# yavuzmurattas/Infrared-Colorization-with-ResNet-Generator-and-PatchGAN

Measured on AMD Instinct MI355X. Metric: GAN train-step img/s (G+D fwd/bwd) at 256×256, 1/2/4/8 MI355X, higher is better.
Workload: dtype bf16; 1 GPU; GAN train step 256x256, batch 16/GPU, bf16 (BASELINE configs[1]); global_batch=16, img_size=256, height=256, width=256, parallelism=dp1

## Files before the change

### include/irgan.h

```cpp
#ifndef IRGAN_H
#define IRGAN_H
#include <stdint.h>
#include <stddef.h>

#if defined(__GNUC__) || defined(__clang__)
#define IRGAN_API __attribute__((visibility("default")))
#else
#define IRGAN_API
#endif

#ifdef __cplusplus
extern "C" {
#endif

typedef void* irgan_stream_t;

IRGAN_API int irgan_build_id(char* buf, int32_t len);

enum { IRGAN_F32 = 0, IRGAN_BF16 = 1, IRGAN_FP8 = 2 };
enum { IRGAN_PAD_ZERO = 0, IRGAN_PAD_REFLECT = 1 };
enum { IRGAN_ACT_NONE = 0, IRGAN_ACT_RELU = 1, IRGAN_ACT_LRELU = 2, IRGAN_ACT_TANH = 3 };
enum { IRGAN_OK = 0, IRGAN_EINVAL = 1001, IRGAN_EUNSUPPORTED = 1002 };

typedef struct irgan_conv_desc {
// ... 31 lines not shown
IRGAN_API int irgan_fp8_quant(const void* x, int32_t dt, int64_t P, int32_t C, int32_t ldx, int32_t xoff,
                    void* y, int32_t ldy, int32_t yoff, const float* q, uint32_t* amax,
                    irgan_stream_t s);
IRGAN_API int irgan_fp8_scale(uint32_t* amax, int32_t n, float* q, float* dq, int32_t reset, irgan_stream_t s);
typedef struct irgan_fp8_job {
    const void* src;
    void* dst;
    int64_t n;
    int32_t slot, reserved;
} irgan_fp8_job;
IRGAN_API int irgan_fp8_quant_batch(const void* jobs, int32_t njobs, int64_t max_n, const float* q,
                          uint32_t* amax, irgan_stream_t s);

IRGAN_API int irgan_conv_fwd_splitk(const irgan_conv_desc* d, const void* x, const void* w, float* y,
                          int32_t ksplit, int64_t split_stride, irgan_stream_t s);

IRGAN_API int irgan_conv_wgrad(const irgan_conv_desc* d, const void* x, const void* dy,
                     float* dw, int32_t splitk, irgan_stream_t s);

IRGAN_API int irgan_conv_wgrad_ws(const irgan_conv_desc* d, const void* x, const void* dy, float* dw,
                        int32_t splitk, float* ws, int64_t ws_floats, irgan_stream_t s);

IRGAN_API int irgan_weight_pack(const float* src, void* dst, int32_t dtype, int32_t Cout, int32_t KH,
                      int32_t KW, int32_t Cin, int32_t transpose, int32_t s, int32_t tyr,
                      int32_t Ay, int32_t txr, int32_t Ax, int32_t cpad, int32_t kalign,
                      irgan_stream_t st);

typedef struct irgan_pack_desc {
    const float* src;
    void* dst;
    int32_t dtype, Cout, KH, KW, Cin, transpose, s, tyr, Ay, txr, Ax, cpad, kalign, reserved;
} irgan_pack_desc;
IRGAN_API int irgan_weight_pack_batch(const irgan_pack_desc* descs, int32_t n, irgan_stream_t st);

enum { IRGAN_IN_PARTS = 256 };
IRGAN_API int irgan_in_finalize(const void* part, int32_t N, int32_t HW, int32_t C, int32_t nb, float* mr,
                      irgan_stream_t s);
IRGAN_API int irgan_in_stats(const void* x, int32_t dtype, int32_t N, int32_t HW, int32_t C,
                   int32_t ld, int32_t off, double* work, float* mr, irgan_stream_t s);
IRGAN_API int irgan_in_apply(const void* x, int32_t dtype, int32_t N, int32_t HW, int32_t C, int32_t ldx,
                   int32_t xoff, const float* mr, int32_t act, const void* res, int32_t ldr,
                   int32_t roff, void* y, int32_t ldy, int32_t yoff, void* xhat, irgan_stream_t s);
IRGAN_API int irgan_in_bwd_reduce(const void* dy, int32_t dy_dtype, int32_t lddy, int32_t dyoff,
                        const void* dy2, int32_t dy2_dtype, int32_t lddy2, int32_t dy2off,
                        const void* x, int32_t x_dtype, int32_t ldx, int32_t xoff, int32_t act,
                        int32_t N, int32_t HW, int32_t C, const float* mr, double* work,
                        float* red, irgan_stream_t s);
IRGAN_API int irgan_in_bwd_apply(const void* dy, int32_t dy_dtype, int32_t lddy, int32_t dyoff,
                       const void* dy2, int32_t dy2_dtype, int32_t lddy2, int32_t dy2off,
                       const void* x, int32_t x_dtype, int32_t ldx, int32_t xoff, int32_t act,
                       int32_t N, int32_t HW, int32_t C, const float* mr, const float* red,
                       void* dx, int32_t dx_dtype, int32_t lddx, int32_t dxoff, float* db,
                       irgan_stream_t s);

IRGAN_API int irgan_in_apply_fp8(const void* x, int32_t N, int32_t HW, int32_t C, int32_t ldx, int32_t xoff,
                       const float* mr, int32_t act, const void* res, int32_t ldr, int32_t roff, void* y,
                       int32_t ldy, int32_t yoff, void* y8, int32_t ld8, int32_t off8, const float* q,
                       uint32_t* amax, irgan_stream_t s);
IRGAN_API int irgan_in_bwd_apply_fp8(const void* dy, int32_t lddy, int32_t dyoff, const void* dy2, int32_t lddy2,
                           int32_t dy2off, const void* x, int32_t ldx, int32_t xoff, int32_t act, int32_t N,
                           int32_t HW, int32_t C, const float* mr, const float* red, void* dx, int32_t lddx,
                           int32_t dxoff, void* y8, int32_t ld8, int32_t off8, const float* q,
                           uint32_t* amax, irgan_stream_t s);
IRGAN_API int irgan_channel_sum(const void* g, int32_t dtype, int32_t P, int32_t C, int32_t ld,
                      int32_t off, float* db, double* work, irgan_stream_t s);

enum { IRGAN_BN_TABLE = 4 };
enum { IRGAN_NORM_AFFINE = 256 };
IRGAN_API int irgan_bn_finalize(const void* part, int32_t N, int32_t HW, int32_t C, int32_t nb, int32_t G,
                      const float* gamma, const float* beta, float* running_mean, float* running_var,
                      float momentum, float eps, int32_t repeat, float* mr, float* ab, irgan_stream_t s);
IRGAN_API int irgan_bn_stats(const void* x, int32_t dtype, int32_t N, int32_t HW, int32_t C, int32_t ld,
                   int32_t off, int32_t G, const float* gamma, const float* beta, float* running_mean,
                   float* running_var, float momentum, float eps, int32_t repeat, double* work, float* mr,
                   float* ab, irgan_stream_t s);
IRGAN_API int irgan_bn_eval_table(const float* running_mean, const float* running_var, const float* gamma,
                        const float* beta, int32_t N, int32_t C, float eps, float* mr, float* ab,
                        irgan_stream_t s);
IRGAN_API int irgan_bn_apply(const void* x, int32_t dtype, int32_t N, int32_t HW, int32_t C, int32_t ldx,
                   int32_t xoff, const float* mr, const float* gamma, const float* beta, int32_t act,
                   const void* res, int32_t ldr, int32_t roff, void* y, int32_t ldy, int32_t yoff,
                   irgan_stream_t s);
IRGAN_API int irgan_bn_backward(const void* dy, int32_t dy_dtype, int32_t lddy, int32_t dyoff, const void* dy2,
                      int32_t dy2_dtype, int32_t lddy2, int32_t dy2off, const void* x, int32_t x_dtype,
                      int32_t ldx, int32_t xoff, int32_t act, int32_t N, int32_t HW, int32_t C, int32_t G,
                      int32_t eval, const float* mr, const float* gamma, const float* beta, double* work,
                      float* red, void* dx, int32_t dx_dtype, int32_t lddx, int32_t dxoff, float* dgamma,
                      float* dbeta, irgan_stream_t s);

IRGAN_API int irgan_resample_table(int32_t kind, int32_t n_in, int32_t p, int32_t transpose, int32_t* idx,
                         float* w, int32_t tmax, int32_t rows_cap);
IRGAN_API int irgan_reflect_ring_fold(const float* rows, const float* cols, int32_t nsplit, int32_t N, int32_t H,
                            int32_t W, int32_t C, int32_t p, void* dx, int32_t dx_dtype, int32_t lddx,
                            int32_t dxoff, irgan_stream_t s);
IRGAN_API int irgan_reflect_dgrad_ring(const irgan_conv_desc* d, const void* dy, const void* w, int32_t p, void* dx,
                             irgan_stream_t s);
IRGAN_API int irgan_reflect_dgrad_ring_ws(const irgan_conv_desc* d, const void* dy, const void* w, int32_t p, void* dx,
                                float* ws, int64_t ws_floats, int32_t max_blocks, irgan_stream_t s);
IRGAN_API int irgan_conv_dgrad_reflect_line(const irgan_conv_desc* d, const void* dy, const void* w, int32_t p, void* dx,
                                  float* ws, int64_t ws_floats, irgan_stream_t s);
IRGAN_API int irgan_conv_dgrad_reflect_line_fp8(const irgan_conv_desc* d, const void* dy, const void* w,
                                      const irgan_conv_desc* d8, const void* dy8, const void* w8,
                                      const float* dqy, const float* dqw, int32_t p, void* dx, float* ws,
                                      int64_t ws_floats, irgan_stream_t s);
IRGAN_API int irgan_conv_dgrad_s2(const irgan_conv_desc* d, const void* dy, const void* const* w, void* dx,
                        const void* mask, irgan_stream_t s);
IRGAN_API int irgan_sep_resample(const void* in, int32_t in_dtype, int32_t N, int32_t Hin, int32_t Win,
                       int32_t C, int32_t ldi, int32_t offi, void* out, int32_t out_dtype,
                       int32_t Hout, int32_t Wout, int32_t ldo, int32_t offo, const int32_t* ty,
                       const float* wy, int32_t Ty, const int32_t* tx, const float* wx,
                       int32_t Tx, int32_t accumulate, irgan_stream_t s);
IRGAN_API int irgan_sep_resample_in(const void* in, int32_t in_dtype, int32_t N, int32_t Hin, int32_t Win,
                          int32_t C, int32_t ldi, int32_t offi, const float* mr, int32_t act,
                          void* out, int32_t out_dtype, int32_t Hout, int32_t Wout, int32_t ldo,
                          int32_t offo, const int32_t* ty, const float* wy, int32_t Ty,
                          const int32_t* tx, const float* wx, int32_t Tx, irgan_stream_t s);
// ... 87 lines not shown
```

### infrared-colorization-with-resnet-generator-and-patchgan_amd/csrc/common.h

```cpp
#pragma once
#include <hip/hip_runtime.h>
#include <stdint.h>
#include <stdlib.h>
#include "irgan.h"

typedef uint16_t bf16_t;
typedef __attribute__((ext_vector_type(8))) __bf16 bf16x8_t;
typedef __attribute__((ext_vector_type(4))) float f32x4;

#define IRGAN_HD __device__ __forceinline__


IRGAN_HD float bf2f(bf16_t v) { return __uint_as_float(((uint32_t)v) << 16); }
IRGAN_HD bf16_t f2bf(float f) { return __builtin_bit_cast(bf16_t, (__bf16)f); }
IRGAN_HD uint32_t pk_bf16(float lo, float hi) {
    typedef __bf16 bf16x2_t __attribute__((ext_vector_type(2)));
    const bf16x2_t v = {(__bf16)lo, (__bf16)hi};
    return __builtin_bit_cast(uint32_t, v);
}

IRGAN_HD float ldv(const void* p, int dt, int64_t i) {
    return dt == IRGAN_BF16 ? bf2f(((const bf16_t*)p)[i]) : ((const float*)p)[i];
}
IRGAN_HD void stv(void* p, int dt, int64_t i, float v) {
// ... 39 lines not shown

IRGAN_HD void glds16(const void* src, const void* lds) {
    const uint32_t m = (uint32_t)(uintptr_t)(__attribute__((address_space(3))) const char*)lds;
    asm volatile("s_nop 0\n\tglobal_load_lds_dwordx4 %0, off" ::"v"(src), "{m0}"(m) : "memory");
}
typedef int32_t i32x4 __attribute__((ext_vector_type(4)));
IRGAN_HD i32x4 make_rsrc(const void* base, uint32_t bytes) {
    const uint64_t a = (uint64_t)(uintptr_t)base;
    i32x4 r;
    r.x = (int32_t)(uint32_t)a;
    r.y = (int32_t)(uint32_t)(a >> 32);
    r.z = (int32_t)bytes;
    r.w = 0x00020000;
    return r;
}
constexpr uint32_t IRGAN_OOB = 0x80000000u;
constexpr int IRGAN_RING_ROWS = 68;
IRGAN_HD void blds16(i32x4 rsrc, uint32_t voff, const void* lds) {
    const uint32_t m = (uint32_t)(uintptr_t)(__attribute__((address_space(3))) const char*)lds;
    asm volatile("s_nop 0\n\tbuffer_load_dwordx4 %0, %1, 0 offen lds" ::"v"(voff), "s"(rsrc), "{m0}"(m) : "memory");
}
IRGAN_HD void blds16(i32x4 rsrc, uint32_t voff, uint32_t soff, const void* lds) {
    const uint32_t m = (uint32_t)(uintptr_t)(__attribute__((address_space(3))) const char*)lds;
    asm volatile("s_nop 0\n\tbuffer_load_dwordx4 %0, %1, %2 offen lds" ::"v"(voff), "s"(rsrc), "s"(soff), "{m0}"(m)
                 : "memory");
}
template <int N>
IRGAN_HD void wait_vmcnt() {
    static_assert(N >= 0 && N <= 63, "vmcnt");
    asm volatile("s_waitcnt vmcnt(%0)" ::"n"(N) : "memory");
}
template <int M>
IRGAN_HD float dpp_xor16(float v) {
    int x = __float_as_int(v);
    if constexpr (M == 1) {
        x = __builtin_amdgcn_update_dpp(0, x, 0xB1, 0xF, 0xF, false);
    } else if constexpr (M == 2) {
        x = __builtin_amdgcn_update_dpp(0, x, 0x4E, 0xF, 0xF, false);
    } else if constexpr (M == 4) {
        x = __builtin_amdgcn_update_dpp(0, x, 0x141, 0xF, 0xF, false);
        x = __builtin_amdgcn_update_dpp(0, x, 0x1B, 0xF, 0xF, false);
    } else {
        static_assert(M == 8, "dpp_xor16: M in {1, 2, 4, 8}");
        x = __builtin_amdgcn_update_dpp(0, x, 0x128, 0xF, 0xF, false);
    }
    return __int_as_float(x);
}
IRGAN_HD void lds_barrier() { asm volatile("s_barrier" ::: "memory"); }

IRGAN_HD int xcd_tile(int b, int nb, int swz) {
    if (!swz || (nb & 7)) return b;
    return (b & 7) * (nb >> 3) + (b >> 3);
}

#define IRGAN_LAUNCH_CHECK()                    \
    do {                                          \
        hipError_t e__ = hipGetLastError();       \
        if (e__ != hipSuccess) return (int)e__;   \
    } while (0)

static inline int irgan_cdiv(long a, long b) { return (int)((a + b - 1) / b); }

constexpr int IRGAN_MAX_DEVICES = 64;
static inline int irgan_device() {
    int d = 0;
    return (hipGetDevice(&d) == hipSuccess && d >= 0 && d < IRGAN_MAX_DEVICES) ? d : -1;
}
static inline int irgan_cu_count() {
    static int cache[IRGAN_MAX_DEVICES];
    const int dev = irgan_device();
    if (dev < 0) return 256;
    int c = __atomic_load_n(&cache[dev], __ATOMIC_RELAXED);
    if (!c) {
        if (hipDeviceGetAttribute(&c, hipDeviceAttributeMultiprocessorCount, dev) != hipSuccess || c < 1) c = 256;
        __atomic_store_n(&cache[dev], c, __ATOMIC_RELAXED);
    }
    return c;
}
static inline void* irgan_symbol(const void* sym, void** cache) {
    const int dev = irgan_device();
    if (dev < 0) return nullptr;
    void* p = __atomic_load_n(&cache[dev], __ATOMIC_ACQUIRE);
    if (!p) {
        if (hipGetSymbolAddress(&p, sym) != hipSuccess) return nullptr;
        __atomic_store_n(&cache[dev], p, __ATOMIC_RELEASE);
    }
    return p;
}
static inline bool irgan_det(const irgan_conv_desc* d) { return (d->flags & IRGAN_CONV_DETERMINISTIC) != 0; }
static inline int irgan_xcd_swz() {
    static const int v = getenv("IRGAN_NO_XCD_SWZ") ? 0 : 1;
    return v;
}
```

### infrared-colorization-with-resnet-generator-and-patchgan_amd/csrc/conv_wgrad_pc.hip

```cpp
#include "common.h"

#ifndef PC_EXP
#define PC_EXP 0
#endif
#define PCX(b) ((PC_EXP & (b)) != 0)

namespace {

typedef __attribute__((ext_vector_type(4))) short s16x4;
typedef __attribute__((address_space(3))) s16x4 lds_s4;

IRGAN_HD int pc_t128(int r) { return ((r >> 1) & 1) | (((r >> 3) & 1) << 1); }
IRGAN_HD int pc_t256(int r) { return (r & 3) | (((r >> 3) & 1) << 2); }

constexpr int XPIECES = 9;
#ifndef WGPC_LW
#define WGPC_LW 4
#endif
#ifndef WGPC_STAGES
#define WGPC_STAGES 4
#endif
template <int BMC>
constexpr int stages_of() { return BMC == 128 ? WGPC_STAGES : 4; }
static_assert(WGPC_STAGES >= 4, "the schedule needs segment k-1's stage free after barrier k");
// ... 217 lines not shown
#if !PCX(8)
        lds_barrier();
#endif
        __builtin_amdgcn_sched_barrier(0);
    };
    Frag<MI, NJ> f0, f1;
#if PCX(32)
    __builtin_amdgcn_s_setprio(1);
#endif
    barrier();
    {
        const char* S = smem;
#pragma unroll
        for (int i = 0; i < MI; ++i) f0.a[i] = ld_tr_pair(S + aoff[i], S + aoff[i] + 4 * DYR);
#pragma unroll
        for (int j = 0; j < NJ; ++j) f0.b[j] = ld_tr_pair(S + boff[j][0][0], S + boff[j][1][0]);
    }
    for (int kt = 0; kt < nk; ++kt) {
        step(f0, f1, kt % STAGES, 1);
        barrier();
        step(f1, f0, (kt + 1) % STAGES, 0);
    }

    const int K = d.KH * KW * d.Cin;
    float* const dst = slab ? slab + (long)split * d.Cout * K : nullptr;
#pragma unroll
    for (int i = 0; i < MI; ++i)
#pragma unroll
        for (int rr = 0; rr < 4; ++rr) {
            const int co = co0 + (wm * MI + i) * 16 + g * 4 + rr;
            if (co >= d.Cout) continue;
#pragma unroll
            for (int j = 0; j < NJ; ++j) {
                const int jj = wn * NJ + j, tx = jj >> 2;
                const int ci = ci0 + (jj & 3) * 16 + (lane & 15);
                const long o = (long)co * K + (ty * KW + tx) * d.Cin + ci;
                if (dst) dst[o] = acc[i][j][rr];
                else atomicAdd(dw + o, acc[i][j][rr]);
            }
        }
}

constexpr int W2_AP = 16;
constexpr int W2_XP = 2 * XPIECES;
constexpr int W2_TP = W2_AP + W2_XP;
constexpr int W2_STAGE = W2_TP * 1024;
constexpr int W2_LW = 4, W2_CW = 8, W2_NT = (W2_CW + W2_LW) * 64;
constexpr int W2_PPL = (W2_TP + W2_LW - 1) / W2_LW;
constexpr int W2_STAGES = 4;
#ifndef W2_EXP
#define W2_EXP 0
#endif

IRGAN_HD int xcd_tile_any(int b, int nb) {
    const int x = b & 7, k = b >> 3, per = nb >> 3, rem = nb & 7;
    return x * per + (x < rem ? x : rem) + k;
}

__global__ __launch_bounds__(W2_NT, 1) void wgrad_w2_kernel(const irgan_conv_desc d, const bf16_t* __restrict__ x,
                                                            const bf16_t* __restrict__ dy, float* __restrict__ dw,
                                                            int segs_per_block, int nseg, int ntco, int nci2, int swz,
                                                            float* __restrict__ slab) {
    constexpr int DYR = 256, MI = 4, NJ = 6;
    __shared__ __attribute__((aligned(1024))) char smem[W2_STAGES * W2_STAGE];
    const int tid = threadIdx.x, lane = tid & 63;
    const int wid = __builtin_amdgcn_readfirstlane(tid >> 6);
    const int tiles = ntco * nci2 * d.KH;
    const int t = swz ? xcd_tile_any(blockIdx.x, gridDim.x) : blockIdx.x;
    const int split = t / tiles;
    int r = t - split * tiles;
    const int ty = r % d.KH;
    r /= d.KH;
    const int cic = r % nci2, cot = r / nci2;
    const int co0 = cot * 128, ci0 = cic * 128;
    const int s_beg = split * segs_per_block;
    const int s_end = min(nseg, s_beg + segs_per_block);
    if (s_beg >= s_end) return;
    const int nk = s_end - s_beg;
    const int segs_row = (d.Wo + 63) / 64;

    if (wid >= W2_CW) {
        const int l = wid - W2_CW;
        const int np = (W2_TP - l + W2_LW - 1) / W2_LW;
        const bool reflect = d.pad_mode == IRGAN_PAD_REFLECT;
        const i32x4 rs_dy = make_rsrc(dy + d.yoff + co0,
                                      (uint32_t)(((long)d.N * d.Ho * d.Wo * d.ldy - d.yoff - co0) * 2));
        const i32x4 rs_x = make_rsrc(x + d.xoff + ci0, (uint32_t)(((long)d.N * d.H * d.W * d.ldx - d.xoff - ci0) * 2));
        uint32_t voff[W2_PPL];
        int xpos[W2_PPL], xc16[W2_PPL];
#pragma unroll
        for (int u = 0; u < W2_PPL; ++u) {
            const int j = l + W2_LW * u;
            voff[u] = IRGAN_OOB;
            xpos[u] = 0;
            xc16[u] = 0;
            if (j < W2_AP) {
                const int pos = j * 4 + lane / 16, slot = lane % 16;
                const int c16 = slot ^ (2 * pc_t256(pos));
                voff[u] = (uint32_t)((pos * d.ldy + c16 * 8) * 2);
                xpos[u] = pos;
            } else if (j < W2_TP) {
                const int jx = j - W2_AP, plane = jx / XPIECES;
                const int pos = (jx - plane * XPIECES) * 8 + (lane >> 3), slot = lane & 7;
                xpos[u] = pos;
                xc16[u] = ((slot ^ (2 * pc_t128(pos))) * 8 + plane * 64) * 2;
            }
        }
        auto issue = [&](int s, int stage) {
            const int rowi = s / segs_row;
            const int x0 = (s - rowi * segs_row) * 64;
            const int n = rowi / d.Ho, oy = rowi - n * d.Ho;
// ... 196 lines not shown
```

### infrared-colorization-with-resnet-generator-and-patchgan_amd/csrc/norm.hip

```cpp
#include "fp8_util.h"

namespace {

struct Q8 {
    uint8_t* p;
    int ld, off;
    const float* q;
    uint32_t* amax;
};

constexpr int TPB = 256;
constexpr int V = 8;
constexpr int IN_PARTS = 128;

IRGAN_HD void ld8(const void* p, int dt, long i, float* o) {
    if (dt == IRGAN_BF16) {
        const uint4 u = *(const uint4*)((const bf16_t*)p + i);
        const uint32_t w[4] = {u.x, u.y, u.z, u.w};
#pragma unroll
        for (int k = 0; k < 4; ++k) {
            o[2 * k] = __uint_as_float(w[k] << 16);
            o[2 * k + 1] = __uint_as_float(w[k] & 0xffff0000u);
        }
    } else {
// ... 486 lines not shown
int rp_of(int C, int VW) {
    int cl = (C + VW - 1) / VW;
    if (cl > TPB) cl = TPB;
    return TPB / cl;
}

int blocks_per_image(long HW, int N, int RP, long rpt = 8) {
    long nb = (4096 + N - 1) / (N > 0 ? N : 1);
    const long maxnb = (HW + rpt * RP - 1) / (rpt * RP);
    if (nb > maxnb) nb = maxnb;
    if (nb > IN_PARTS) nb = IN_PARTS;
    if (nb < 1) nb = 1;
    return (int)nb;
}

template <int MODE>
int launch_rows(Slice X, Slice DY, Slice DY2, int act, const float* mr, const float* red, void* dx, int dxdt, int lddx,
                int dxoff, int N, int HW, int C, float2* part, float* db, bool vec, hipStream_t st, int* nb_out,
                const Q8* q8 = nullptr) {
    const int VW = vec ? V : 1;
    const int rpt = pass_rpt(MODE, PASS_RPT[MODE]);
    const int RP = rp_of(C, VW);
    int nb = blocks_per_image(HW, N, RP, rpt);
    const int rows = irgan_cdiv(HW, nb);
    nb = irgan_cdiv(HW, rows);
    const int rpth = irgan_cdiv(rows, RP);
    dim3 g(nb, N);
    static const bool fast = !getenv("IRGAN_NO_ROWS8");
    const bool bf = X.dt == IRGAN_BF16 && (MODE == 0 || (DY.dt == IRGAN_BF16 && (!DY2.p || DY2.dt == IRGAN_BF16))) &&
                    (MODE != 2 || (dxdt == IRGAN_BF16 && !db));
    if (q8 && !(vec && bf && MODE == 2)) return IRGAN_EUNSUPPORTED;
    if ((fast || q8) && vec && bf && MODE <= 2) {
        const bf16_t *xp = (const bf16_t*)X.p, *gp = (const bf16_t*)DY.p, *hp = (const bf16_t*)DY2.p;
        if (MODE == 2 && q8)
            rows8_go<2, true>(2, rpth, g, st, xp, X.ld, X.off, gp, DY.ld, DY.off, hp, DY2.ld, DY2.off, act, mr, red,
                              (bf16_t*)dx, lddx, dxoff, HW, C, rows, part, *q8);
        else if (MODE == 0)
            rows8_go<0>(0, rpth, g, st, xp, X.ld, X.off, (const bf16_t*)nullptr, 0, 0, (const bf16_t*)nullptr, 0, 0, act, mr,
                        red, (bf16_t*)nullptr, 0, 0, HW, C, rows, part, Q8{});
        else
            rows8_go<MODE>(MODE, rpth, g, st, xp, X.ld, X.off, gp, DY.ld, DY.off, hp, DY2.ld, DY2.off, act, mr, red,
                           (bf16_t*)dx, lddx, dxoff, HW, C, rows, part, Q8{});
        if (nb_out) *nb_out = nb;
        return 0;
    }
    if (vec)
        rows_kernel<MODE, V><<<g, TPB, 0, st>>>(X, DY, DY2, act, mr, red, dx, dxdt, lddx, dxoff, HW, C, rows, part, db);
    else
        rows_kernel<MODE, 1><<<g, TPB, 0, st>>>(X, DY, DY2, act, mr, red, dx, dxdt, lddx, dxoff, HW, C, rows, part, db);
    if (nb_out) *nb_out = nb;
    return 0;
}

}

extern "C" int irgan_in_stats(const void* x, int32_t dtype, int32_t N, int32_t HW, int32_t C, int32_t ld,
                              int32_t off, double* work, float* mr, irgan_stream_t s) {
    hipStream_t st = (hipStream_t)s;
    if ((long)N * HW * C <= 0) return 0;
    Slice X{x, dtype, ld, off}, Z{nullptr, 0, 0, 0};
    int nb = 1;
    launch_rows<0>(X, Z, Z, 0, nullptr, nullptr, nullptr, 0, 0, 0, N, HW, C, (float2*)work, nullptr,
                   vec_ok(C, {ld, off}), st, &nb);
    finalize_kernel<<<dim3(irgan_cdiv(C, FC), N), 256, 0, st>>>((const float2*)work, mr, N, C, nb, HW, 0);
    IRGAN_LAUNCH_CHECK();
    return 0;
}

extern "C" int irgan_in_finalize(const void* part, int32_t N, int32_t HW, int32_t C, int32_t nb, float* mr,
                                 irgan_stream_t s) {
    if ((long)N * HW * C <= 0) return 0;
    if (!part || !mr || nb < 1 || nb > IRGAN_IN_PARTS) return IRGAN_EINVAL;
    finalize_kernel<<<dim3(irgan_cdiv(C, FC), N), 256, 0, (hipStream_t)s>>>((const float2*)part, mr, N, C, nb, HW, 0);
    IRGAN_LAUNCH_CHECK();
    return 0;
}



bool apply_rows(const void* x, int ldx, int xoff, int N, int HW, int C, const float* mr, int act, const void* res,
                int ldr, int roff, void* y, int ldy, int yoff, hipStream_t st, const Q8* q8 = nullptr) {
    static const bool off = getenv("IRGAN_NO_APPLY_ROWS") != nullptr;
    if (off) return false;
    const int key = res || q8 ? 5 : 4;
    const int rpt = pass_rpt(key, PASS_RPT[key]);
    const int RP = rp_of(C, 8);
    int nb = blocks_per_image(HW, N, RP, rpt);
    const int rows = irgan_cdiv(HW, nb);
    nb = irgan_cdiv(HW, rows);
    const int rpth = irgan_cdiv(rows, RP);
    dim3 g(nb, N);
    const bf16_t *xp = (const bf16_t*)x, *rp = (const bf16_t*)res;
    if (q8)
        rows8_go<4, true>(key, rpth, g, st, xp, ldx, xoff, rp, ldr, roff, (const bf16_t*)nullptr, 0, 0, act, mr,
                          (const float*)nullptr, (bf16_t*)y, ldy, yoff, HW, C, rows, (float2*)nullptr, *q8);
    else
        rows8_go<4>(key, rpth, g, st, xp, ldx, xoff, rp, ldr, roff, (const bf16_t*)nullptr, 0, 0, act, mr,
                    (const float*)nullptr, (bf16_t*)y, ldy, yoff, HW, C, rows, (float2*)nullptr, Q8{});
    return true;
}

extern "C" int irgan_in_apply(const void* x, int32_t dtype, int32_t N, int32_t HW, int32_t C, int32_t ldx,
                              int32_t xoff, const float* mr, int32_t act, const void* res, int32_t ldr, int32_t roff,
                              void* y, int32_t ldy, int32_t yoff, void* xhat, irgan_stream_t s) {
    const bool vec = vec_ok(C, {ldx, xoff, ldy, yoff}) && (!res || vec_ok(C, {ldr, roff}));
    if (vec && dtype == IRGAN_BF16 && !xhat && (long)N * HW * C > 0 &&
        apply_rows(x, ldx, xoff, N, HW, C, mr, act, res, ldr, roff, y, ldy, yoff, (hipStream_t)s)) {
        IRGAN_LAUNCH_CHECK();
        return 0;
    }
    const int VW = vec ? V : 1;
    long total = (long)N * HW * (C / VW);
    if (total <= 0) return 0;
    int blocks = (int)std::min<long>((total + TPB - 1) / TPB, 16384);
    Slice X{x, dtype, ldx, xoff}, R{res, dtype, ldr, roff};
    if (vec)
        apply_kernel<V><<<blocks, TPB, 0, (hipStream_t)s>>>(X, HW, C, mr, act, R, y, ldy, yoff, xhat, total);
    else
        apply_kernel<1><<<blocks, TPB, 0, (hipStream_t)s>>>(X, HW, C, mr, act, R, y, ldy, yoff, xhat, total);
    IRGAN_LAUNCH_CHECK();
    return 0;
}

extern "C" int irgan_in_bwd_reduce(const void* dy, int32_t dy_dtype, int32_t lddy, int32_t dyoff, const void* dy2,
                                   int32_t dy2_dtype, int32_t lddy2, int32_t dy2off, const void* x, int32_t x_dtype,
                                   int32_t ldx, int32_t xoff, int32_t act, int32_t N, int32_t HW, int32_t C,
                                   const float* mr, double* work, float* red, irgan_stream_t s) {
    hipStream_t st = (hipStream_t)s;
    if ((long)N * HW * C <= 0) return 0;
    const bool vec = vec_ok(C, {lddy, dyoff, ldx, xoff}) && (!dy2 || vec_ok(C, {lddy2, dy2off}));
    Slice X{x, x_dtype, ldx, xoff}, DY{dy, dy_dtype, lddy, dyoff}, DY2{dy2, dy2_dtype, lddy2, dy2off};
    int nb = 1;
    launch_rows<1>(X, DY, DY2, act, mr, nullptr, nullptr, 0, 0, 0, N, HW, C, (float2*)work, nullptr, vec, st, &nb);
    finalize_kernel<<<dim3(irgan_cdiv(C, FC), N), 256, 0, st>>>((const float2*)work, red, N, C, nb, HW, 1);
    IRGAN_LAUNCH_CHECK();
    return 0;
}

extern "C" int irgan_in_bwd_apply(const void* dy, int32_t dy_dtype, int32_t lddy, int32_t dyoff, const void* dy2,
                                  int32_t dy2_dtype, int32_t lddy2, int32_t dy2off, const void* x, int32_t x_dtype,
                                  int32_t ldx, int32_t xoff, int32_t act, int32_t N, int32_t HW, int32_t C,
                                  const float* mr, const float* red, void* dx, int32_t dx_dtype, int32_t lddx,
                                  int32_t dxoff, float* db, irgan_stream_t s) {
    const bool vec = vec_ok(C, {lddy, dyoff, ldx, xoff, lddx, dxoff}) && (!dy2 || vec_ok(C, {lddy2, dy2off}));
    Slice X{x, x_dtype, ldx, xoff}, DY{dy, dy_dtype, lddy, dyoff}, DY2{dy2, dy2_dtype, lddy2, dy2off};
    launch_rows<2>(X, DY, DY2, act, mr, red, dx, dx_dtype, lddx, dxoff, N, HW, C, nullptr, db, vec, (hipStream_t)s,
                   nullptr);
    IRGAN_LAUNCH_CHECK();
    return 0;
}

static __global__ __launch_bounds__(256) void colsum_finalize_kernel(const float2* __restrict__ part, float* __restrict__ db,
                                                              int nb, int C) {
    __shared__ double sp[FS][FC];
    const int cl = threadIdx.x % FC, sub = threadIdx.x / FC, c = blockIdx.x * FC + cl;
    double t = 0.0;
    if (c < C)
        for (int b = sub; b < nb; b += FS) t += part[(long)b * C + c].x;
    sp[sub][cl] = t;
    __syncthreads();
    if (sub != 0 || c >= C) return;
    t = 0.0;
    for (int k = 0; k < FS; ++k) t += sp[k][cl];
    db[c] += (float)t;
}

extern "C" int irgan_channel_sum(const void* g, int32_t dtype, int32_t P, int32_t C, int32_t ld, int32_t off,
                                 float* db, double* work, irgan_stream_t s) {
    if (P <= 0) return 0;
    hipStream_t st = (hipStream_t)s;
    Slice X{g, dtype, ld, off}, Z{nullptr, 0, 0, 0};
    int S = 16;
    while (S > 1 && (P % S || P / S < 4096)) S >>= 1;
    int nb = 1;
    launch_rows<0>(X, Z, Z, 0, nullptr, nullptr, nullptr, 0, 0, 0, S, P / S, C, (float2*)work, nullptr,
                   vec_ok(C, {ld, off}), st, &nb);
    colsum_finalize_kernel<<<irgan_cdiv(C, FC), 256, 0, st>>>((const float2*)work, db, S * nb, C);
    IRGAN_LAUNCH_CHECK();
    return 0;
}

extern "C" int irgan_in_apply_fp8(const void* x, int32_t N, int32_t HW, int32_t C, int32_t ldx, int32_t xoff,
                                  const float* mr, int32_t act, const void* res, int32_t ldr, int32_t roff, void* y,
                                  int32_t ldy, int32_t yoff, void* y8, int32_t ld8, int32_t off8, const float* q,
                                  uint32_t* amax, irgan_stream_t s) {
    if (!x || !mr || !y || !y8 || !q || !amax) return IRGAN_EINVAL;
    if (!vec_ok(C, {ldx, xoff, ldy, yoff, ld8, off8}) || (res && !vec_ok(C, {ldr, roff}))) return IRGAN_EUNSUPPORTED;
    const long total = (long)N * HW * (C / V);
    if (total <= 0) return 0;
    const Q8 q8v{(uint8_t*)y8, ld8, off8, q, amax};
    if (apply_rows(x, ldx, xoff, N, HW, C, mr, act, res, ldr, roff, y, ldy, yoff, (hipStream_t)s, &q8v)) {
        IRGAN_LAUNCH_CHECK();
        return 0;
    }
    const int blocks = (int)std::min<long>((total + TPB - 1) / TPB, 16384);
    Slice X{x, IRGAN_BF16, ldx, xoff}, R{res, IRGAN_BF16, ldr, roff};
    apply_kernel<V, true><<<blocks, TPB, 0, (hipStream_t)s>>>(X, HW, C, mr, act, R, y, ldy, yoff, nullptr, total,
                                                               q8v);
    IRGAN_LAUNCH_CHECK();
    return 0;
}

extern "C" int irgan_in_bwd_apply_fp8(const void* dy, int32_t lddy, int32_t dyoff, const void* dy2, int32_t lddy2,
                                      int32_t dy2off, const void* x, int32_t ldx, int32_t xoff, int32_t act, int32_t N,
// ... 16 lines not shown
```

### infrared-colorization-with-resnet-generator-and-patchgan_amd/ops.py

```python
from __future__ import annotations

import ctypes
import math
import os

import torch

from . import _lib
from ._lib import (ACT_LRELU, ACT_NONE, ACT_RELU, ACT_TANH, BF16, F32, FP8, IN_PARTS, PAD_REFLECT,
                   PAD_ZERO)

TORCH_DT = {F32: torch.float32, BF16: torch.bfloat16, FP8: torch.float8_e4m3fn}


def dt_code(t: torch.Tensor) -> int:
    if t.dtype == torch.float32:
        return F32
    if t.dtype == torch.bfloat16:
        return BF16
    if t.dtype == torch.float8_e4m3fn:
        return FP8
    raise TypeError(f"unsupported dtype {t.dtype}")


# ... 461 lines not shown


def _wgrad_ws(dev):
    key = (dev, torch.cuda.current_stream(dev).cuda_stream)
    w = _WGRAD_WS.get(key)
    if w is None:
        w = _WGRAD_WS[key] = torch.empty(WGRAD_WS_FLOATS, dtype=torch.float32, device=dev)
    return w



def in_stats(x: Feat, work: torch.Tensor, mr: torch.Tensor):
    _lib.call("irgan_in_stats", x.ptr, x.dt, x.N, x.H * x.W, x.C, x.ld, x.off, P(work), P(mr), stream())


def in_finalize(x: Feat, part: torch.Tensor, nb: int, mr: torch.Tensor):
    _lib.call("irgan_in_finalize", P(part), x.N, x.H * x.W, x.C, nb, P(mr), stream())


def in_apply(x: Feat, mr, y: Feat, act=ACT_NONE, res: Feat = None, xhat: torch.Tensor = None, q8=None):
    assert x.dt == y.dt
    if q8 is not None:
        y8, qp, ap = q8
        assert xhat is None and x.dt == BF16 and y8.dt == FP8 and (y8.N, y8.H, y8.W, y8.C) == (y.N, y.H, y.W, y.C)
        _lib.call("irgan_in_apply_fp8", x.ptr, x.N, x.H * x.W, x.C, x.ld, x.off, P(mr), act,
                  res.ptr if res else None, res.ld if res else 0, res.off if res else 0, y.ptr, y.ld, y.off,
                  y8.ptr, y8.ld, y8.off, qp, ap, stream())
        return
    _timed("in_apply_res" if res is not None else "in_apply", x, lambda: _lib.call(
        "irgan_in_apply", x.ptr, x.dt, x.N, x.H * x.W, x.C, x.ld, x.off, P(mr), act, res.ptr if res else None,
        res.ld if res else 0, res.off if res else 0, y.ptr, y.ld, y.off, P(xhat), stream()))


def in_bwd_parts(dy: Feat, x: Feat, act: int, mr, work, red, dx: Feat, db=None, dy2: Feat = None, q8=None):
    N, HW, C = x.N, x.H * x.W, x.C
    d2 = (dy2.ptr, dy2.dt, dy2.ld, dy2.off) if dy2 is not None else (None, 0, 0, 0)

    def reduce():
        _lib.call("irgan_in_bwd_reduce", dy.ptr, dy.dt, dy.ld, dy.off, *d2, x.ptr, x.dt, x.ld, x.off, act, N, HW, C,
                  P(mr), P(work), P(red), stream())

    def apply():
        if q8 is not None:
            y8, qp, ap = q8
            assert db is None and y8.dt == FP8 and dx.dt == BF16 and (y8.N, y8.H, y8.W, y8.C) == (dx.N, dx.H, dx.W, C)
            _lib.call("irgan_in_bwd_apply_fp8", dy.ptr, dy.ld, dy.off, d2[0], d2[2], d2[3], x.ptr, x.ld, x.off, act,
                      N, HW, C, P(mr), P(red), dx.ptr, dx.ld, dx.off, y8.ptr, y8.ld, y8.off, qp, ap, stream())
            return
        _lib.call("irgan_in_bwd_apply", dy.ptr, dy.dt, dy.ld, dy.off, *d2, x.ptr, x.dt, x.ld, x.off, act, N, HW, C,
                  P(mr), P(red), dx.ptr, dx.dt, dx.ld, dx.off, P(db), stream())
    return reduce, apply


def in_backward(dy: Feat, x: Feat, act: int, mr, work, red, dx: Feat, db=None, dy2: Feat = None, q8=None):
    reduce, apply = in_bwd_parts(dy, x, act, mr, work, red, dx, db, dy2, q8)
    _timed("in_bwd_reduce", x, reduce)
    _timed("in_bwd_apply", x, apply)


_CS_WORK = {}


def channel_sum(g: Feat, db: torch.Tensor):
    key = (db.device, g.C, torch.cuda.current_stream(db.device).cuda_stream)
    w = _CS_WORK.get(key)
    if w is None:
        w = _CS_WORK[key] = torch.empty(16 * IN_PARTS * g.C, dtype=torch.float64, device=db.device)
    _lib.call("irgan_channel_sum", g.ptr, g.dt, g.P, g.C, g.ld, g.off, P(db), P(w), stream())



NORM_AFFINE = _lib.header_enum("IRGAN_NORM_AFFINE")
BN_TABLE = _lib.header_enum("IRGAN_BN_TABLE")
BN_EPS, BN_MOMENTUM = 1e-5, 0.1


def bn_stats(x: Feat, work: torch.Tensor, mr: torch.Tensor, groups=1, gamma=None, beta=None, running_mean=None,
             running_var=None, repeat=1, ab=None, nb=0):
    assert x.N % groups == 0 and repeat >= 1
    if nb:
        _lib.call("irgan_bn_finalize", P(work), x.N, x.H * x.W, x.C, nb, groups, P(gamma), P(beta), P(running_mean),
                  P(running_var), BN_MOMENTUM, BN_EPS, repeat, P(mr), P(ab), stream())
    else:
        _lib.call("irgan_bn_stats", x.ptr, x.dt, x.N, x.H * x.W, x.C, x.ld, x.off, groups, P(gamma), P(beta),
                  P(running_mean), P(running_var), BN_MOMENTUM, BN_EPS, repeat, P(work), P(mr), P(ab), stream())


def bn_eval_table(running_mean, running_var, gamma, beta, N: int, mr: torch.Tensor, ab=None):
    _lib.call("irgan_bn_eval_table", P(running_mean), P(running_var), P(gamma), P(beta), N, running_mean.numel(),
              BN_EPS, P(mr), P(ab), stream())


def bn_apply(x: Feat, mr, gamma, beta, y: Feat, act=ACT_NONE, res: Feat = None):
    assert x.dt == y.dt and (res is None or res.dt == x.dt)
    _lib.call("irgan_bn_apply", x.ptr, x.dt, x.N, x.H * x.W, x.C, x.ld, x.off, P(mr), P(gamma), P(beta), act,
              res.ptr if res else None, res.ld if res else 0, res.off if res else 0, y.ptr, y.ld, y.off, stream())


def bn_backward(dy: Feat, x: Feat, act: int, mr, gamma, beta, work, red, dx: Feat, dgamma=None, dbeta=None, groups=1,
                eval_mode=False, dy2: Feat = None):
    d2 = (dy2.ptr, dy2.dt, dy2.ld, dy2.off) if dy2 is not None else (None, 0, 0, 0)
    _lib.call("irgan_bn_backward", dy.ptr, dy.dt, dy.ld, dy.off, *d2, x.ptr, x.dt, x.ld, x.off, act, x.N, x.H * x.W,
              x.C, groups, int(eval_mode), P(mr), P(gamma), P(beta), P(work), P(red), dx.ptr, dx.dt, dx.ld, dx.off,
              P(dgamma), P(dbeta), stream())



# ... 450 lines not shown
```

Measured before the change: 1304 img/s.

## Fuse instance-norm backward reduce and apply into a single-pass kernel

Adds a one-pass instance-norm backward kernel. It keeps each block's x and dy tiles in registers, reduces the per-channel gradient sums inside the block, and writes dx, with optional fp8 quantization, without a second global read. This removes one kernel launch and a re-read of x and dy for small-spatial layers where one image×channel-group fits in a block. It only applies when HW*16 is at most 65536 and there are enough blocks to fill the CUs, and it falls back to the two-kernel path otherwise. The cost is one block per image×channel-group, which may limit parallelism, and heavy register use.

```diff
diff --git a/include/irgan.h b/include/irgan.h
--- a/include/irgan.h
+++ b/include/irgan.h
@@ -107,6 +107,13 @@
                        int32_t N, int32_t HW, int32_t C, const float* mr, const float* red,
                        void* dx, int32_t dx_dtype, int32_t lddx, int32_t dxoff, float* db,
                        irgan_stream_t s);
+enum { IRGAN_IN_ONEPASS_CG = 16, IRGAN_IN_ONEPASS_ELEMS = 65536 };
+IRGAN_API int irgan_in_bwd_onepass(const void* dy, int32_t dy_dtype, int32_t lddy, int32_t dyoff,
+                         const void* dy2, int32_t dy2_dtype, int32_t lddy2, int32_t dy2off,
+                         const void* x, int32_t x_dtype, int32_t ldx, int32_t xoff, int32_t act,
+                         int32_t N, int32_t HW, int32_t C, const float* mr, float* red,
+                         void* dx, int32_t dx_dtype, int32_t lddx, int32_t dxoff,
+                         irgan_stream_t s);
 
 IRGAN_API int irgan_in_apply_fp8(const void* x, int32_t N, int32_t HW, int32_t C, int32_t ldx, int32_t xoff,
                        const float* mr, int32_t act, const void* res, int32_t ldr, int32_t roff, void* y,
@@ -117,6 +124,11 @@
                            int32_t HW, int32_t C, const float* mr, const float* red, void* dx, int32_t lddx,
                            int32_t dxoff, void* y8, int32_t ld8, int32_t off8, const float* q,
                            uint32_t* amax, irgan_stream_t s);
+IRGAN_API int irgan_in_bwd_onepass_fp8(const void* dy, int32_t lddy, int32_t dyoff, const void* dy2, int32_t lddy2,
+                             int32_t dy2off, const void* x, int32_t ldx, int32_t xoff, int32_t act, int32_t N,
+                             int32_t HW, int32_t C, const float* mr, float* red, void* dx, int32_t lddx,
+                             int32_t dxoff, void* y8, int32_t ld8, int32_t off8, const float* q,
+                             uint32_t* amax, irgan_stream_t s);
 IRGAN_API int irgan_channel_sum(const void* g, int32_t dtype, int32_t P, int32_t C, int32_t ld,
                       int32_t off, float* db, double* work, irgan_stream_t s);
 
diff --git a/infrared-colorization-with-resnet-generator-and-patchgan_amd/csrc/common.h b/infrared-colorization-with-resnet-generator-and-patchgan_amd/csrc/common.h
--- a/infrared-colorization-with-resnet-generator-and-patchgan_amd/csrc/common.h
+++ b/infrared-colorization-with-resnet-generator-and-patchgan_amd/csrc/common.h
@@ -115,6 +115,10 @@
     if (!swz || (nb & 7)) return b;
     return (b & 7) * (nb >> 3) + (b >> 3);
 }
+IRGAN_HD int xcd_tile_any(int b, int nb) {
+    const int x = b & 7, k = b >> 3, per = nb >> 3, rem = nb & 7;
+    return x * per + (x < rem ? x : rem) + k;
+}
 
 #define IRGAN_LAUNCH_CHECK()                    \
     do {                                          \
diff --git a/infrared-colorization-with-resnet-generator-and-patchgan_amd/csrc/conv_wgrad_pc.hip b/infrared-colorization-with-resnet-generator-and-patchgan_amd/csrc/conv_wgrad_pc.hip
--- a/infrared-colorization-with-resnet-generator-and-patchgan_amd/csrc/conv_wgrad_pc.hip
+++ b/infrared-colorization-with-resnet-generator-and-patchgan_amd/csrc/conv_wgrad_pc.hip
@@ -293,11 +293,6 @@
 #define W2_EXP 0
 #endif
 
-IRGAN_HD int xcd_tile_any(int b, int nb) {
-    const int x = b & 7, k = b >> 3, per = nb >> 3, rem = nb & 7;
-    return x * per + (x < rem ? x : rem) + k;
-}
-
 __global__ __launch_bounds__(W2_NT, 1) void wgrad_w2_kernel(const irgan_conv_desc d, const bf16_t* __restrict__ x,
                                                             const bf16_t* __restrict__ dy, float* __restrict__ dw,
                                                             int segs_per_block, int nseg, int ntco, int nci2, int swz,
diff --git a/infrared-colorization-with-resnet-generator-and-patchgan_amd/csrc/norm.hip b/infrared-colorization-with-resnet-generator-and-patchgan_amd/csrc/norm.hip
--- a/infrared-colorization-with-resnet-generator-and-patchgan_amd/csrc/norm.hip
+++ b/infrared-colorization-with-resnet-generator-and-patchgan_amd/csrc/norm.hip
@@ -562,6 +562,203 @@
     return 0;
 }
 
+#ifndef IN_ONEPASS_CG
+#define IN_ONEPASS_CG IRGAN_IN_ONEPASS_CG
+#endif
+constexpr int OP_CG = IN_ONEPASS_CG;
+constexpr int OP_MAXU = 16;
+constexpr int OP_MAXNT = 512;
+constexpr int OP_CAP = IRGAN_IN_ONEPASS_ELEMS;
+
+template <bool F8, int NT, int CG, int U>
+__global__ __launch_bounds__(NT) void in_bwd_onepass_kernel(const bf16_t* x, int ldx, int xoff, const bf16_t* dy,
+                                                            int lddy, int dyoff, int act,
+                                                            const float* __restrict__ mr, float* __restrict__ red,
+                                                            bf16_t* dx, int lddx, int dxoff, int HW, int C, int swz,
+                                                            int nb, int rows, int RP, Q8 q8) {
+    constexpr int LPP = CG / 8, NCH = NT / LPP;
+    static_assert(LPP == 1 || LPP == 2 || LPP == 4, "CG in {8, 16, 32}");
+    __shared__ float sc[NCH][CG * 2];
+    __shared__ float pt[IN_PARTS][CG * 2];
+    __shared__ float sf[CG][2];
+    const int G = C / CG;
+    const int t = swz ? xcd_tile_any(blockIdx.x, gridDim.x) : blockIdx.x;
+    const int n = t / G, cg = t - n * G;
+    const int h = threadIdx.x % LPP, q = threadIdx.x / LPP;
+    const int b = q / RP, rl = q - b * RP;
+    const bool on = q < nb * RP;
+    const int r0 = b * rows + rl, r1 = on ? min(HW, (b + 1) * rows) : 0;
+    const long pb = (long)n * HW;
+    const bf16_t* xb = x + pb * ldx + xoff + cg * CG;
+    const bf16_t* gb = dy + pb * lddy + dyoff + cg * CG;
+    bf16_t* ob = dx + pb * lddx + dxoff + cg * CG;
+    const uint32_t h8 = h * 8;
+
+    uint4 xr[U], gr[U];
+#pragma unroll
+    for (int u = 0; u < U; ++u) {
+        const uint32_t p = min(r0 + u * RP, HW - 1);
+        xr[u] = *(const uint4*)(xb + (p * (uint32_t)ldx + h8));
+        gr[u] = *(const uint4*)(gb + (p * (uint32_t)lddy + h8));
+    }
+    typedef const float __attribute__((address_space(4))) * cfloat_p;
+    const cfloat_p mrow = (cfloat_p)(uintptr_t)(mr + 2 * ((long)n * C + cg * CG));
+    float mean[8], rstd[8];
+#pragma unroll
+    for (int k = 0; k < 8; ++k) {
+        mean[k] = mrow[2 * k];
+        rstd[k] = mrow[2 * k + 1];
+#pragma unroll
+        for (int j = 1; j < LPP; ++j) {
+            mean[k] = h == j ? mrow[2 * (j * 8 + k)] : mean[k];
+            rstd[k] = h == j ? mrow[2 * (j * 8 + k) + 1] : rstd[k];
+        }
+    }
+    const float neg = act == IRGAN_ACT_RELU ? 0.f : act == IRGAN_ACT_LRELU ? 0.2f : 1.f;
+    float a0[8], a1[8];
+#pragma unroll
+    for (int k = 0; k < 8; ++k) { a0[k] = 0.f; a1[k] = 0.f; }
+#pragma unroll
+    for (int u = 0; u < U; ++u) {
+        if (r0 + u * RP >= r1) gr[u] = make_uint4(0u, 0u, 0u, 0u);
+        float xv[8], gv[8];
+        bf8f(xr[u], xv);
+        bf8f(gr[u], gv);
+#pragma unroll
+        for (int k = 0; k < 8; ++k) {
+            const float xh = (xv[k] - mean[k]) * rstd[k];
+            const float f = xh > 0.f ? 1.f : neg;
+            a0[k] = __builtin_fmaf(gv[k], f, a0[k]);
+            a1[k] = __builtin_fmaf(gv[k] * f, xh, a1[k]);
+        }
+        __builtin_amdgcn_sched_barrier(0);
+    }
+#pragma unroll
+    for (int k = 0; k < 8; ++k) {
+        sc[q][(h * 8 + k) * 2] = a0[k];
+        sc[q][(h * 8 + k) * 2 + 1] = a1[k];
+    }
+    __syncthreads();
+    const int CL = min(C / 8, TPB);
+    const bool tree = CL <= 64 && (64 % CL) == 0;
+    for (int task = threadIdx.x; task < nb * CG * 2; task += NT) {
+        const int cw = task % (CG * 2), pbk = task / (CG * 2);
+        const int c0 = pbk * RP;
+        float tsum = 0.f;
+        if (tree) {
+            const int RW = RP / (TPB / 64);
+            for (int j = 0; j < TPB / 64; ++j) {
+                for (int o = 1; o < RW; o <<= 1)
+                    for (int i = 0; i < RW; i += 2 * o) sc[c0 + j * RW + i][cw] += sc[c0 + j * RW + i + o][cw];
+                tsum += sc[c0 + j * RW][cw];
+            }
+        } else {
+            for (int j = 0; j < RP; ++j) tsum += sc[c0 + j][cw];
+        }
+        pt[pbk][cw] = tsum;
+    }
+    __syncthreads();
+    if (threadIdx.x < CG * 2) {
+        const int cw = threadIdx.x;
+        double s = 0.0;
+        for (int k = 0; k < FS; ++k) {
+            double l = 0.0;
+            for (int pbk = k; pbk < nb; pbk += FS) l += pt[pbk][cw];
+            s += l;
+        }
+        const float v = (float)(s / HW);
+        sf[cw >> 1][cw & 1] = v;
+        red[2 * ((long)n * C + cg * CG) + cw] = v;
+    }
+    __syncthreads();
+    float mg[8], mgx[8];
+#pragma unroll
+    for (int k = 0; k < 8; ++k) { mg[k] = sf[h * 8 + k][0]; mgx[k] = sf[h * 8 + k][1]; }
+
+    const float qs = F8 ? *q8.q : 1.f;
+    float amx = 0.f;
+    uint8_t* qb = F8 ? q8.p + pb * q8.ld + q8.off + cg * CG : nullptr;
+#pragma unroll
+    for (int u = 0; u < U; ++u) {
+        asm volatile("" : "+v"(xr[u].x), "+v"(xr[u].y), "+v"(xr[u].z), "+v"(xr[u].w));
+        asm volatile("" : "+v"(gr[u].x), "+v"(gr[u].y), "+v"(gr[u].z), "+v"(gr[u].w));
+        const uint32_t p = r0 + u * RP;
+        if ((int)p >= r1) break;
+        float xv[8], gv[8], o[8];
+        bf8f(xr[u], xv);
+        bf8f(gr[u], gv);
+#pragma unroll
+        for (int k = 0; k < 8; ++k) {
+            const float xh = (xv[k] - mean[k]) * rstd[k];
+            const float f = xh > 0.f ? 1.f : neg;
+            o[k] = rstd[k] * __builtin_fmaf(-xh, mgx[k], __builtin_fmaf(gv[k], f, -mg[k]));
+        }
+        uint4 w;
+        w.x = pk_bf16(o[0], o[1]);
+        w.y = pk_bf16(o[2], o[3]);
+        w.z = pk_bf16(o[4], o[5]);
+        w.w = pk_bf16(o[6], o[7]);
+        *(uint4*)(ob + (p * (uint32_t)lddx + h8)) = w;
+        if constexpr (F8) {
+            float vb[8];
+            bf8f(w, vb);
+#pragma unroll
+            for (int k = 0; k < 8; ++k) amx = fmaxf(amx, fabsf(vb[k]));
+            *(uint2*)(qb + (p * (uint32_t)q8.ld + h8)) = pack8_fp8(vb, qs);
+        }
+        __builtin_amdgcn_sched_barrier(0);
+    }
+    if constexpr (F8) fp8_block_amax(amx, q8.amax, blockIdx.x);
+}
+
+struct OnepassPlan {
+    int nb, rows, RP, chain, threads;
+};
+bool onepass_plan(int N, int HW, int C, OnepassPlan* pl) {
+    pl->RP = rp_of(C, 8);
+    int nb = blocks_per_image(HW, N, pl->RP, pass_rpt(1, PASS_RPT[1]));
+    pl->rows = irgan_cdiv(HW, nb);
+    pl->nb = irgan_cdiv(HW, pl->rows);
+    pl->chain = irgan_cdiv(pl->rows, pl->RP);
+    pl->threads = pl->nb * pl->RP * (OP_CG / 8);
+    return pl->chain <= OP_MAXU && pl->threads <= OP_MAXNT && pl->nb <= IN_PARTS;
+}
+
+bool onepass_ok(int N, int HW, int C, std::initializer_list<int> lds) {
+    if (N < 0 || HW < 0 || C < 0 || C % OP_CG || (long)HW * OP_CG > OP_CAP) return false;
+    for (int l : lds)
+        if (l % 8 || l < 0 || (long)HW * l >= (1L << 30)) return false;
+    OnepassPlan pl;
+    return (long)N * HW * C <= 0 || onepass_plan(N, HW, C, &pl);
+}
+
+template <bool F8, int NT>
+void onepass_nt(const OnepassPlan& pl, dim3 g, hipStream_t st, const bf16_t* x, int ldx, int xoff, const bf16_t* dy,
+                int lddy, int dyoff, int act, const float* mr, float* red, bf16_t* dx, int lddx, int dxoff, int HW,
+                int C, Q8 q8) {
+    const int swz = irgan_xcd_swz();
+#define OP_GO(U_)                                                                                                    \
+    in_bwd_onepass_kernel<F8, NT, OP_CG, U_><<<g, NT, 0, st>>>(x, ldx, xoff, dy, lddy, dyoff, act, mr, red, dx, lddx, \
+                                                                dxoff, HW, C, swz, pl.nb, pl.rows, pl.RP, q8)
+    if (pl.chain <= 1) OP_GO(1);
+    else if (pl.chain <= 2) OP_GO(2);
+    else if (pl.chain <= 4) OP_GO(4);
+    else if (pl.chain <= 8) OP_GO(8);
+    else OP_GO(16);
+#undef OP_GO
+}
+
+template <bool F8>
+void onepass_go(const bf16_t* x, int ldx, int xoff, const bf16_t* dy, int lddy, int dyoff, int act, const float* mr,
+                float* red, bf16_t* dx, int lddx, int dxoff, int N, int HW, int C, hipStream_t st, Q8 q8) {
+    OnepassPlan pl;
+    onepass_plan(N, HW, C, &pl);
+    const dim3 g(N * (C / OP_CG));
+    if (pl.threads <= 128) onepass_nt<F8, 128>(pl, g, st, x, ldx, xoff, dy, lddy, dyoff, act, mr, red, dx, lddx, dxoff, HW, C, q8);
+    else if (pl.threads <= 256) onepass_nt<F8, 256>(pl, g, st, x, ldx, xoff, dy, lddy, dyoff, act, mr, red, dx, lddx, dxoff, HW, C, q8);
+    else onepass_nt<F8, 512>(pl, g, st, x, ldx, xoff, dy, lddy, dyoff, act, mr, red, dx, lddx, dxoff, HW, C, q8);
+}
+
 }
 
 extern "C" int irgan_in_stats(const void* x, int32_t dtype, int32_t N, int32_t HW, int32_t C, int32_t ld,
@@ -660,6 +857,38 @@
     return 0;
 }
 
+extern "C" int irgan_in_bwd_onepass(const void* dy, int32_t dy_dtype, int32_t lddy, int32_t dyoff, const void* dy2,
+                                    int32_t dy2_dtype, int32_t lddy2, int32_t dy2off, const void* x, int32_t x_dtype,
+                                    int32_t ldx, int32_t xoff, int32_t act, int32_t N, int32_t HW, int32_t C,
+                                    const float* mr, float* red, void* dx, int32_t dx_dtype, int32_t lddx,
+                                    int32_t dxoff, irgan_stream_t s) {
+    (void)dy2_dtype; (void)lddy2; (void)dy2off;
+    if (!dy || !x || !mr || !red || !dx) return IRGAN_EINVAL;
+    if (dy2 || dy_dtype != IRGAN_BF16 || x_dtype != IRGAN_BF16 || dx_dtype != IRGAN_BF16 ||
+        !onepass_ok(N, HW, C, {lddy, dyoff, ldx, xoff, lddx, dxoff}))
+        return IRGAN_EUNSUPPORTED;
+    if ((long)N * HW * C <= 0) return 0;
+    onepass_go<false>((const bf16_t*)x, ldx, xoff, (const bf16_t*)dy, lddy, dyoff, act, mr, red, (bf16_t*)dx, lddx,
+                      dxoff, N, HW, C, (hipStream_t)s, Q8{});
+    IRGAN_LAUNCH_CHECK();
+    return 0;
+}
+
+extern "C" int irgan_in_bwd_onepass_fp8(const void* dy, int32_t lddy, int32_t dyoff, const void* dy2, int32_t lddy2,
+                                        int32_t dy2off, const void* x, int32_t ldx, int32_t xoff, int32_t act,
+                                        int32_t N, int32_t HW, int32_t C, const float* mr, float* red, void* dx,
+                                        int32_t lddx, int32_t dxoff, void* y8, int32_t ld8, int32_t off8,
+                                        const float* q, uint32_t* amax, irgan_stream_t s) {
+    (void)lddy2; (void)dy2off;
+    if (!dy || !x || !mr || !red || !dx || !y8 || !q || !amax) return IRGAN_EINVAL;
+    if (dy2 || !onepass_ok(N, HW, C, {lddy, dyoff, ldx, xoff, lddx, dxoff, ld8, off8})) return IRGAN_EUNSUPPORTED;
+    if ((long)N * HW * C <= 0) return 0;
+    onepass_go<true>((const bf16_t*)x, ldx, xoff, (const bf16_t*)dy, lddy, dyoff, act, mr, red, (bf16_t*)dx, lddx,
+                     dxoff, N, HW, C, (hipStream_t)s, Q8{(uint8_t*)y8, ld8, off8, q, amax});
+    IRGAN_LAUNCH_CHECK();
+    return 0;
+}
+
 static __global__ __launch_bounds__(256) void colsum_finalize_kernel(const float2* __restrict__ part, float* __restrict__ db,
                                                               int nb, int C) {
     __shared__ double sp[FS][FC];
diff --git a/infrared-colorization-with-resnet-generator-and-patchgan_amd/ops.py b/infrared-colorization-with-resnet-generator-and-patchgan_amd/ops.py
--- a/infrared-colorization-with-resnet-generator-and-patchgan_amd/ops.py
+++ b/infrared-colorization-with-resnet-generator-and-patchgan_amd/ops.py
@@ -537,7 +537,57 @@
     return reduce, apply
 
 
+IN_ONEPASS_CG = _lib.header_enum("IRGAN_IN_ONEPASS_CG")
+IN_ONEPASS_ELEMS = _lib.header_enum("IRGAN_IN_ONEPASS_ELEMS")
+IN_BWD_ONEPASS = [os.environ.get("IRGAN_IN_BWD_ONEPASS") != "0"]
+_CUS = {}
+
+
+def _cu_count(dev) -> int:
+    c = _CUS.get(dev)
+    if c is None:
+        c = _CUS[dev] = torch.cuda.get_device_properties(dev).multi_processor_count
+    return c
+
+
+def in_bwd_onepass_legal(N, HW, C, dts, lds, has_db=False, has_dy2=False) -> bool:
+    return (all(d == BF16 for d in dts) and not has_db and not has_dy2 and C % IN_ONEPASS_CG == 0
+            and HW * IN_ONEPASS_CG <= IN_ONEPASS_ELEMS and all(v % 8 == 0 for v in lds))
+
+
+def in_bwd_use_onepass(N, HW, C, dts, lds, cus, has_db=False, has_dy2=False, q8=None) -> bool:
+    del q8
+    return (IN_BWD_ONEPASS[0] and in_bwd_onepass_legal(N, HW, C, dts, lds, has_db, has_dy2)
+            and 2 * N * (C // IN_ONEPASS_CG) >= cus)
+
+
+def in_bwd_onepass(dy: Feat, x: Feat, act: int, mr, red, dx: Feat, dy2: Feat = None, q8=None) -> bool:
+    N, HW, C = x.N, x.H * x.W, x.C
+    d2 = (dy2.ptr, dy2.dt, dy2.ld, dy2.off) if dy2 is not None else (None, 0, 0, 0)
+    lib = _lib.load()
+    if q8 is not None:
+        y8, qp, ap = q8
+        if not (dy.dt == x.dt == dx.dt == BF16 and (dy2 is None or dy2.dt == BF16)):
+            return False
+        assert y8.dt == FP8 and (y8.N, y8.H, y8.W, y8.C) == (dx.N, dx.H, dx.W, C)
+        rc = lib.irgan_in_bwd_onepass_fp8(dy.ptr, dy.ld, dy.off, d2[0], d2[2], d2[3], x.ptr, x.ld, x.off, act, N, HW,
+                                          C, P(mr), P(red), dx.ptr, dx.ld, dx.off, y8.ptr, y8.ld, y8.off, qp, ap,
+                                          stream())
+    else:
+        rc = lib.irgan_in_bwd_onepass(dy.ptr, dy.dt, dy.ld, dy.off, *d2, x.ptr, x.dt, x.ld, x.off, act, N, HW, C,
+                                      P(mr), P(red), dx.ptr, dx.dt, dx.ld, dx.off, stream())
+    if rc == IRGAN_EUNSUPPORTED:
+        return False
+    if rc != 0:
+        raise _lib.IrganError(f"irgan_in_bwd_onepass failed with code {rc}")
+    return True
+
+
 def in_backward(dy: Feat, x: Feat, act: int, mr, work, red, dx: Feat, db=None, dy2: Feat = None, q8=None):
+    if in_bwd_use_onepass(x.N, x.H * x.W, x.C, (dy.dt, x.dt, dx.dt), (dy.ld, dy.off, x.ld, x.off, dx.ld, dx.off),
+                          _cu_count(x.t.device), db is not None, dy2 is not None, q8):
+        if _timed("in_bwd_apply", x, lambda: in_bwd_onepass(dy, x, act, mr, red, dx, q8=q8)):
+            return
     reduce, apply = in_bwd_parts(dy, x, act, mr, work, red, dx, db, dy2, q8)
     _timed("in_bwd_reduce", x, reduce)
     _timed("in_bwd_apply", x, apply)
```

Measured after the change: 1322 img/s, median of 6. 1.01x the previous value.
